# baoe/AlignGraph

Measured on AMD Instinct MI355X. Metric: aligned reads/sec through graph build+extend, higher is better.
Workload: dtype u32

## Files before the change

### aligngraph_amd/csrc/agx_core.h

```cpp
#pragma once
#include <stdint.h>
#include "../../include/agx.h"

#if defined(__HIPCC__)
#define AGX_HD __host__ __device__ __forceinline__
#else
#define AGX_HD inline
#endif

typedef uint32_t agx_u32;
typedef uint16_t agx_u16;
typedef uint8_t agx_u8;

#define AGX_NONE 0xFFFFFFFFu
#define AGX_TILE 64u
#ifndef AGX_REGION_TILES
#define AGX_REGION_TILES 32u
#endif
#define AGX_REGION_PAD 32u
#ifndef AGX_MAXV_LDS
#define AGX_MAXV_LDS 2u
#endif
#ifndef AGX_SWEEP_FIRST
#define AGX_SWEEP_FIRST 1
// ... 95 lines not shown
AGX_HD agx_u32 agx_cside_nruns(agx_u32 c) { return (c & 0xFFu) | (c >> 8) << 16; }
AGX_HD agx_u32 agx_cside_total(agx_u32 nruns) { return (nruns & 0xFFFFu) + (nruns >> 16); }
AGX_HD agx_wside agx_cside_rebuild(agx_u32 first, agx_u32 before, agx_u32 nruns) { const agx_u32 n1 = nruns & 0xFFFFu, r1 = first + before; return agx_wside{n1 ? r1 : 0u, (nruns >> 16) ? r1 + n1 : 0u, nruns}; }
AGX_HD bool agx_cside_in_order(const agx_wside &sd, unsigned long long &at) {
    const agx_u32 n1 = sd.nruns & 0xFFFFu, n2 = sd.nruns >> 16;
    const bool fine = sd.runs1 == (n1 ? at : 0ull) && sd.runs2 == (n2 ? at + n1 : 0ull);
    at += n1 + n2;
    return fine && at <= 0xFFFFFFFFull;
}
AGX_HD agx_u32 agx_cside_first(const agx_wside *sides, size_t n) { return !n ? 0u : (sides[0].nruns & 0xFFFFu) ? sides[0].runs1 : (sides[0].nruns >> 16) ? sides[0].runs2 : 0u; }
AGX_HD bool agx_sides_consecutive(const agx_wside *sides, size_t n, agx_u32 &first) {
    first = agx_cside_first(sides, n);
    unsigned long long at = first;
    for (size_t i = 0; i < n; i++) if (!agx_cside_in_order(sides[i], at)) return false;
    return true;
}
struct agx_refx { agx_u32 pos, len, byte; };
AGX_HD agx_u32 agx_ref_code(agx_u32 c) { return c == 'A' ? 0u : c == 'C' ? 1u : c == 'G' ? 2u : c == 'T' ? 3u : 4u; }
AGX_HD char agx_ref_base(agx_u32 code) { return (char)((0x54474341u >> (8u * (code & 3u))) & 0xFFu); }

struct agx_cmkey { agx_u32 cid, coff; };
struct agx_cmhead { agx_u32 cid, coff, n, start; };


enum { AGX_HF_AREV = 1, AGX_HF_SKIP = 2, AGX_HF_BNONE = 4 };

struct agx_dhit {
    agx_u32 a_t0, b_t0;
    agx_u32 a_runs, b_runs;
    agx_u32 a_slot;
// ... 1210 lines not shown
```

### aligngraph_amd/csrc/agx_engine.cpp

```cpp
#include "agx_unit.h"


struct HsaCopy {
    bool ok = false; hsa_agent_t cpu{}; std::vector<hsa_agent_t> gpu; std::vector<std::string> uuid;
    static hsa_status_t on_agent(hsa_agent_t a, void *p) {
        HsaCopy *H = (HsaCopy *)p; hsa_device_type_t t;
        if (hsa_agent_get_info(a, HSA_AGENT_INFO_DEVICE, &t) != HSA_STATUS_SUCCESS) return HSA_STATUS_SUCCESS;
        if (t == HSA_DEVICE_TYPE_CPU && !H->cpu.handle) H->cpu = a;
        if (t == HSA_DEVICE_TYPE_GPU) {
            char id[32] = {0};
            (void)hsa_agent_get_info(a, (hsa_agent_info_t)HSA_AMD_AGENT_INFO_UUID, id);
            H->gpu.push_back(a); H->uuid.push_back(std::string(id, strnlen(id, 21)));
        }
        return HSA_STATUS_SUCCESS;
    }
    HsaCopy() {
        if (getenv("AGX_NO_SDMA_DOWNLOAD")) return;
        if (hsa_init() != HSA_STATUS_SUCCESS) return;
        if (hsa_iterate_agents(on_agent, this) != HSA_STATUS_SUCCESS) return;
        ok = cpu.handle != 0 && !gpu.empty();
    }
    bool agent_of(int device, hsa_agent_t &out) const {
        static std::mutex m; static int known[64]; static hsa_agent_t agent[64];
        std::lock_guard<std::mutex> l(m);
// ... 265 lines not shown
        u->side_first = agx_cside_first(sd, n); unsigned long long at = u->side_first;
        for (size_t i = 0; i < n && fine; i++) { fine = agx_cside_in_order(sd[i], at); listed += agx_cside_pack(sd[i].nruns) == AGX_CS_ESC; }
        const size_t counts_bytes = (n * 2 + 7) & ~(size_t)7, bytes = n * 2 + listed * sizeof(agx_cside_esc);
        if (fine && bytes >= n * sizeof(agx_wside)) fine = false;
        if (fine) {
            u->s_csides.alloc(counts_bytes + (listed + 1) * sizeof(agx_cside_esc));
            agx_u16 *c = (agx_u16 *)u->s_csides.p; agx_cside_esc *l = (agx_cside_esc *)(u->s_csides.p + counts_bytes);
            u->wire_listed = l; u->n_csesc = listed;
            for (size_t i = 0; i < n; i++) { const agx_u32 v = agx_cside_pack(sd[i].nruns); c[i] = (agx_u16)v; if (v == AGX_CS_ESC) *l++ = agx_cside_esc{(agx_u32)i, sd[i].nruns}; }
        }
        if (getenv("AGX_LOAD_TIMING")) fprintf(stderr, "[agx load] compact side records: %.1f ms, 12 -> %.2f bytes per side, %.2f %% listed%s\n", now_ms() - t0, (double)bytes / n,
                                              100.0 * listed / n, fine ? "" : ": not used (the run pool is not in side order, or nothing gained)");
    }
    if (!fine) { u->s_csides.release(); return; }
    u->sides_compact = true;
}

void stage_tiled(agx_unit *u, unsigned threads) {
    u->tiled = false; u->n_other_t = 0; u->slot_row.clear(); u->n_win = 1;
    const size_t nh = u->nh, s4 = u->stride / 4;
    if (u->rows_diffed || getenv("AGX_NO_TILED_UPLOAD") || nh == 0 || u->n_rows == 0) { u->s_hits_t.release(); u->s_codes_t.release(); u->s_other_t.release(); return; }
    const double t0 = now_ms();
    const bool compact = want_compact();
    if (compact) u->s_hits_t.alloc_plain(nh + 1); else u->s_hits_t.alloc(nh + 1);
    u->s_codes_t.alloc(nh * s4 + 16); u->slot_row.resize(nh);
    const agx_whit *wh = u->s_hits.p; const agx_wside *sd = u->s_sides.p; const agx_wrun *wr = u->s_runs.p; const agx_u32 *perm = u->s_perm.p;
    const size_t n_rows = u->n_rows; std::vector<agx_u8> has_other((n_rows + 7) / 8, 0);
    for (size_t j = 0; j < u->n_other; j++) { const size_t r = (size_t)(u->s_other.p[j] / u->stride); if (r < n_rows) has_other[r >> 3] |= (agx_u8)(1u << (r & 7)); }
    auto idx0 = [&](const agx_whit &w) -> agx_u32 {
        if (!(w.flags & AGX_WF_RUNS1)) return w.a;
// ... 47 lines not shown
    const char *env = getenv("AGX_ROW_DIFF");
    const size_t n_pos = u->V.n_pos ? u->V.n_pos : u->T.ref.size();
    if (!env || atoi(env) == 0) return;
    const double t0 = now_ms();
    RowDiffs D;
    if (!build_row_diffs(u->s_hits_t.p, u->nh, u->s_sides.p, u->n_sides, u->s_runs.p, u->n_runs, u->s_codes_t.p, u->nh, u->stride, (const agx_u32 *)u->s_ref.p, n_pos, threads, D, true)) return;
    if (D.n_units * 2 + D.cnt.size() + (D.block_off.size() + D.block_first.size() + D.anchor_bits.size()) * 4 >= u->nh * (u->stride / 4)) return;
    adopt_row_diffs(u, D, threads);
    if (getenv("AGX_LOAD_TIMING")) fprintf(stderr, "[agx load] tile-ordered rows against the reference: %.1f ms, %zu rows (%zu as they are), %.1f -> %.1f bytes per row\n", now_ms() - t0, u->nh, u->n_rows_explicit,
                                          (double)(u->stride / 4), (double)(u->n_units * 2 + u->n_rowcnt + (u->n_blockoff + u->n_blockfirst + u->n_anchor) * 4) / u->nh);
}

void finish_staging(agx_unit *u, unsigned threads_rows, unsigned threads) {
    stage_rows(u, threads_rows);
    stage_order(u, threads);
    stage_tiled(u, threads);
    if (!u->tiled) stage_wire_hits(u, threads);
    stage_wire_sides(u);
    stage_rows_tiled(u, threads);
    u->V.slot_row = u->tiled ? u->slot_row.data() : nullptr;
    reserve_landing(u);
    u->staged = true; u->consumed = false; u->uploaded = false; u->built = false; u->downloaded = false;
}

void stage_inputs(agx_unit *u) {
    if (!u->have_ref || !u->have_threads) throw Error{E_ARG, "reference and contig threads must be set before upload"};
    if (u->consumed && u->pairs_staged) throw Error{E_ARG, "one-shot unit: its staged read alignments were overwritten by the download; load the unit again"};
    const double t0 = now_ms();
    HIP_OK(hipSetDevice(u->prm.device));
    u->cache_map.reset(); u->reads_map.reset();
    const size_t n_pos = u->T.ref.size();
    if (n_pos == 0 || n_pos >= 0xFFFFFF00ull) throw Error{E_ARG, "unit sequence is empty or too long"};
    if (u->T.cm_cnt.size() != n_pos) throw Error{E_ARG, "conti-mer chains were not built"};
    { size_t el = 0; for (const agx_cmseg &g : u->T.segs) el += g.len; if (el != u->T.n_cm) throw Error{E_ARG, "conti-mer runs were not built"}; }
// ... 260 lines not shown
    if (u->prm.flags & AGX_FLAG_KEEP_COUNTS) t(u->d_counts, (size_t)cap * 6);
    if (u->prm.flags & AGX_FLAG_EDGE_SUPPORT) t(u->d_e_cnt, (size_t)cap * AGX_MAXE);
    t(u->d_a_str, ids_cap + 1); t(u->d_a_meta, ids_cap + 16); t(u->d_a_mark, ids_cap + 2); t(u->d_side_xpos, (size_t)cap + 1);
    t(u->d_sp_bits, n_words + 1); t(u->d_sp_cnt, n_words + 1); t(u->d_sp_rank, n_words + 2);
    const size_t nb = (std::max<size_t>(n_pos, n_words) + 1 + 1023) / 1024;
    t(u->d_scan_tmp, 2 * (nb + 1) + 2 * ((nb + 1023) / 1024 + 1) + 16); t(u->d_scan_desc, 3 * scan_desc_of(u, cap));
}
template <class U> void fixed_bufs(U *u, Take &t) {
    const size_t n_pos = u->V.n_pos, nh = u->nh, n_tiles = tiles_of(u), n_regions = regions_of(u);
    t(u->d_cm_start, n_pos + 2); t(u->d_cm, u->n_cm + 1); t(u->d_ref, n_pos + 16); t(u->d_cm_head, n_pos + 1);
    t(u->d_segs, u->n_segs + 1); t(u->d_cntruns, u->n_cntruns + 1); t(u->d_cntchunks, u->n_cntchunks + 1); t(u->d_segchunks, u->n_segchunks + 1); t(u->d_segindex, u->n_segindex + 1);
    t(u->d_runs, u->n_runs + 1); t(u->d_vcodes, codes_bytes(u) * 4 + 16); t(u->d_other, others_up(u) + 1);
    if (u->rows_diffed) { t(u->d_units, u->n_units + 2); t(u->d_rowcnt, u->n_rowcnt); t(u->d_blockoff, u->n_blockoff); t(u->d_blockfirst, u->n_blockfirst); t(u->d_anchor, u->n_anchor); }
    else t(u->d_codes, codes_bytes(u) + 16);
    if (u->hits_compact) { t(u->d_chits, u->n_cblocks + 1); t(u->d_cesc, u->n_cesc + 1); t(u->d_cext, u->n_cext + 1); }
    if (u->sides_compact) { t(u->d_csides, u->n_sides + 1); t(u->d_csesc, u->n_csesc + 1); t(u->d_cside_scan, agx_side_scan_words(u->n_sides)); }
    t(u->d_whits, nh + 1); t(u->d_wsides, u->n_sides + 1); t(u->d_wruns, u->n_runs + 1); t(u->d_jump, u->n_jump + 1);
    if (u->ref_packed) { t(u->d_wref, (n_pos + 3) / 4 + 32); t(u->d_refx, u->n_refx + 1); }
    t(u->d_dhit, nh + 1);
    t(u->d_perm, nh + 1); t(u->d_tfirst, n_tiles + 2); t(u->d_ckey, nh + 1); t(u->d_long, AGX_LONG_MAX);
    t(u->d_tile_cnt, n_tiles + 1); t(u->d_tile_off, n_tiles + 2); t(u->d_cursor, n_tiles + 1);
    t(u->d_words, W_TOTAL);
    t(u->d_chain_end, (size_t)u->n_chain_end + 1);
    t(u->d_node_start, n_pos); t(u->d_node_cnt, n_pos); t(u->d_pos_succ, n_pos); t(u->d_slow_list, n_pos + 64);
    t(u->d_side_pk, n_pos + 2); t(u->d_tile_side, n_tiles + 2); t(u->d_tile_side_start, n_tiles + 2);
    t(u->d_big_list, n_tiles + 1); t(u->d_mid_list, n_tiles + 1);
    t(u->d_scratch, (size_t)AGX_BIG_WAVES * AGX_NF * AGX_MAXV_BIG * 64);
    t(u->d_region_off, n_regions + 1); t(u->d_pool_cnt, n_regions * AGX_REGION_PAD);
    if (u->prm.flags & AGX_FLAG_EDGE_SUPPORT) t(u->d_sup_tot, 2 * n_tiles + 2);
}
template <class U> void list_bufs(U *u, agx_u32 cap, Take &t) { t.note(u->list_cap, cap); t(u->d_unsorted, (size_t)cap + 1); t(u->d_tile_recs, ((size_t)cap + 4) * 8); }
template <class U> void ovf_bufs(U *u, agx_u32 cap, Take &t) { t.note(u->ovf_cap, cap); t(u->d_ovf, cap); t(u->d_a_ovf, (size_t)cap + 1); if (u->prm.flags & AGX_FLAG_EDGE_SUPPORT) t(u->d_ovf_cnt, cap); }
// ... 53 lines not shown
        std::lock_guard<std::mutex> up_turn(turn.up_m);
        u->up_timed = u->ev.all;
        if (u->up_timed) HIP_OK(hipEventRecord(u->ev_up0, st));
        static const size_t chunk = getenv("AGX_UP_CHUNK_MB") ? (size_t)atoi(getenv("AGX_UP_CHUNK_MB")) << 20 : 0;
        size_t sent = 0;
        auto up = [&](void *dst, const void *src, size_t bytes) {
            for (size_t at = 0; at < bytes;) { const size_t m = chunk ? std::min(chunk, bytes - at) : bytes; HIP_OK(hipMemcpyAsync((char *)dst + at, (const char *)src + at, m, hipMemcpyHostToDevice, st)); at += m; }
            sent += bytes;
        };
        up(u->d_segs.p, u->s_segs.p, u->n_segs * sizeof(agx_cmseg)); up(u->d_cntruns.p, u->s_cntruns.p, u->n_cntruns * sizeof(agx_cntrun));
        up(u->d_cntchunks.p, u->s_cntchunks.p, u->n_cntchunks * sizeof(agx_chunk)); up(u->d_segchunks.p, u->s_segchunks.p, u->n_segchunks * sizeof(agx_chunk)); up(u->d_segindex.p, u->s_segindex.p, u->n_segindex * 4);
        if (u->hits_compact) { up(u->d_chits.p, u->s_wire.p, u->n_cblocks * sizeof(agx_chit_block)); up(u->d_cesc.p, u->wire_esc, u->n_cesc * sizeof(agx_whit)); up(u->d_cext.p, u->wire_ext, u->n_cext * 4); }
        else up(u->d_whits.p, !u->tiled ? (const void *)u->s_hits.p : u->s_wire.p ? (const void *)u->s_wire.p : (const void *)u->s_hits_t.p, nh * sizeof(agx_whit));
        if (u->sides_compact) { up(u->d_csides.p, u->s_csides.p, u->n_sides * 2); up(u->d_csesc.p, u->wire_listed, u->n_csesc * sizeof(agx_cside_esc)); }
        else up(u->d_wsides.p, u->s_sides.p, u->n_sides * sizeof(agx_wside));
        up(u->d_wruns.p, u->s_runs.p, u->n_runs * sizeof(agx_wrun)); up(u->d_jump.p, u->s_jump_at.p, u->n_jump * 4);
        if (!u->tiled) up(u->d_perm.p, u->s_perm.p, nh * 4);
        up(u->d_tfirst.p, u->s_tfirst.p, ((size_t)u->n_tiles + 2) * 4);
        HIP_OK(hipEventRecord(u->ev_hits, st));
        auto small = [&] {
            up(u->d_other.p, u->tiled ? u->s_other_t.p : u->s_other.p, others_up(u) * 8);
            if (u->ref_packed) { up(u->d_wref.p, u->s_ref.p, (n_pos + 3) / 4); up(u->d_refx.p, u->s_refx.p, u->n_refx * sizeof(agx_refx)); } else up(u->d_ref.p, u->s_ref.p, n_pos);
            up(u->d_chain_end.p, u->s_chain_end.p, (size_t)u->n_chain_end * 4);
            layout_regions(u, nullptr, u->pool_cap - spill_min(u), true, st, &sent);
        };
        auto tables = [&] { up(u->d_blockoff.p, u->s_blockoff.p, u->n_blockoff * 4); up(u->d_blockfirst.p, u->s_blockfirst.p, u->n_blockfirst * 4); up(u->d_anchor.p, u->s_anchor.p, u->n_anchor * 4); };
        if (u->tiled) {
            small();
            if (u->rows_diffed) tables();
            const size_t s4 = u->stride / 4;
            for (agx_u32 w = 0; w < u->n_win; w++) {
// ... 97 lines not shown
        if (attempt > 8) throw Error{E_DEVICE, "build did not converge"};
        const size_t ids_cap = (size_t)n_pos + u->pool_cap;

        const double tb0 = now_ms();
        const bool early = !u->expanded && attempt == 0 && !u->ev.all;
        HIP_OK(wait_event(early ? u->ev_hits : u->ev_uploaded));
        trace(u, "build: wait for upload", tb0, n_pos);
        const double tb1 = now_ms();
        DeviceTurn &turn = turn_of(u->prm.device);
        std::unique_lock<std::mutex> my_turn(turn.m);
        st = turn.front;
        if (turn.n) HIP_OK(hipStreamWaitEvent(st, (u->ev.all || turn.prev_exclusive) ? turn.build_done[(turn.n - 1) & 1] : turn.sweep_done[(turn.n - 1) & 1], 0));
        if (u->ev.all) HIP_OK(hipEventRecord(u->ev.first, st));
        if (!u->expanded) {
            if (u->hits_compact) agx_launch_expand_hits(u->d_chits.p, u->d_cesc.p, u->d_cext.p, u->d_whits.p, nh, u->maxlen, st);
            if (u->sides_compact) agx_launch_expand_sides(u->d_csides.p, u->d_csesc.p, (agx_u32)u->n_csesc, u->d_wsides.p, (agx_u32)u->n_sides, u->side_first, u->d_cside_scan.p, st);
            agx_launch_expand_runs(u->d_wruns.p, u->d_runs.p, (agx_u32)u->n_runs, st);
            agx_launch_cm_tables(u->d_cntruns.p, u->d_cntchunks.p, (agx_u32)u->n_cntchunks, u->d_segs.p, u->d_segchunks.p, (agx_u32)u->n_segchunks, u->d_cm_start.p, u->d_cm.p, u->d_cm_head.p, n_pos, (agx_u32)u->n_cm, st);
        }
        {
            agx_zero_args Z; memset(&Z, 0, sizeof Z);
            auto seg = [&](int i, agx_u32 *ptr, size_t words) { Z.p[i] = ptr; Z.n[i] = (agx_u32)words; };
            seg(0, u->d_words.p, W_TOTAL); seg(1, u->d_tile_cnt.p, (size_t)u->n_tiles + 1); seg(2, u->d_cursor.p, (size_t)u->n_tiles + 1);
            seg(3, u->d_pool_cnt.p, (size_t)u->n_regions * AGX_REGION_PAD); seg(4, u->d_tile_side.p + u->n_tiles, 1); seg(5, u->d_sp_cnt.p, (size_t)u->n_words + 1);
            seg(6, reinterpret_cast<agx_u32 *>(u->d_scan_desc.p), 6 * u->scan_desc_n); seg(7, reinterpret_cast<agx_u32 *>(u->d_sp_bits.p), 2 * ((size_t)u->n_words + 1));
            agx_launch_zero(&Z, st);
            HIP_OK(hipMemsetAsync(u->d_a_mark.p, 0, ids_cap + 2, st));
        }
        u->ev.begin(); u->ev.mark(B_START, st);
        agx_prep_args PA{(const agx_whit *)u->d_whits.p, (const agx_wside *)u->d_wsides.p, u->d_runs.p, u->d_dhit.p, nh, u->prm.k, n_pos, u->d_tile_cnt.p, u->d_words.p + W_ERR,
                         u->d_perm.p, u->d_tfirst.p, u->d_ckey.p, u->lookback, u->d_long.p, u->d_words.p + W_LONGCOUNT, u->tiled ? 1u : 0u, u->d_perm.p};
        agx_launch_hit_prep(&PA, st);
// ... 929 lines not shown
```

### aligngraph_amd/csrc/agx_kargs.h

```cpp
#pragma once
#include <hip/hip_runtime_api.h>
#include "agx_core.h"

struct agx_prep_args {
    const agx_whit *whits; const agx_wside *sides;
    const agx_run *runs; agx_dhit *dhit; agx_u32 n_hits, k, n_pos;
    agx_u32 *tile_cnt;
    agx_u32 *err;
    const agx_u32 *perm, *tile_first; agx_u32 *ckey; agx_u32 lookback; agx_u32 *long_list, *long_count;
    agx_u32 tiled; agx_u32 *perm_out;
};

struct agx_bin_args { const agx_dhit *dhit; agx_u32 n_hits; const agx_u32 *tile_off; agx_u32 *cursor; agx_u32 *unsorted; agx_u32 cap;
                      const agx_u32 *long_count; };

struct agx_node_kargs {
    agx_sweep_args S;
    agx_u32 tile_lo, tile_hi;
    agx_u32 *pool_cnt;
    const agx_u32 *region_off;
    agx_u32 spill_lo; agx_u32 *spill_cnt;
    agx_u32 *mid_count; agx_u32 *mid_list;
    agx_u32 *big_count; agx_u32 *big_list;
    agx_u32 fallback_queued;
// ... 130 lines not shown
#define AGX_SLOW_WAVES 8192u

extern "C" {
struct agx_zero_args { agx_u32 *p[8]; agx_u32 n[8]; };
void agx_launch_zero(const agx_zero_args *, hipStream_t);
void agx_launch_cm_tables(const void *cnt_runs, const void *cnt_chunks, agx_u32 n_cnt_chunks, const agx_cmseg *segs, const void *seg_chunks, agx_u32 n_seg_chunks,
                           agx_u32 *cm_start, agx_cmkey *cm, agx_cmhead *head, agx_u32 n_pos, agx_u32 n_cm, hipStream_t);
void agx_launch_expand_codes(const void *packed, void *vcodes, size_t n_bases16, const unsigned long long *other, size_t n_other, hipStream_t);
void agx_launch_expand_rows(const void *whits, agx_u32 nh, const void *wsides, const void *wruns, const agx_u32 *anchor_bits, const agx_u32 *block_first, const agx_u8 *cnt, const agx_u32 *block_off,
                            const agx_u16 *units, const void *wref, void *vcodes, agx_u32 n_rows, agx_u32 stride, const unsigned long long *other, size_t n_other, hipStream_t);
void agx_launch_patch_codes(const unsigned long long *other, size_t n_other, void *vcodes, hipStream_t);
void agx_launch_expand_runs(const void *wruns, agx_run *runs, agx_u32 n_runs, hipStream_t);
void agx_launch_expand_hits(const agx_chit_block *blocks, const void *esc, const agx_u32 *ext, void *whits, agx_u32 nh, agx_u32 maxlen, hipStream_t);
inline size_t agx_side_scan_words(size_t n) { const size_t nb = (n + 1 + 4095) / 4096, nb2 = (nb + 4095) / 4096; return 2 * (n + 1) + 2 * (nb + 1) + 2 * (nb2 + 1); }
void agx_launch_expand_sides(const agx_u16 *counts, const agx_cside_esc *list, agx_u32 n_list, void *sides, agx_u32 n, agx_u32 first, agx_u32 *scan, hipStream_t);
void agx_launch_expand_ref(const void *packed, void *ref, size_t n_pos16, const void *refx, agx_u32 n_refx, hipStream_t);
void agx_launch_hit_prep(const agx_prep_args *, hipStream_t);
void agx_launch_exclusive_scan(const agx_u32 *in, agx_u32 *out, agx_u32 n, agx_u32 *tmp, hipStream_t);
void agx_launch_exclusive_scan1(const agx_u32 *in, agx_u32 *out, agx_u32 n, unsigned long long *desc, hipStream_t);
void agx_launch_exclusive_scan1_capped(const agx_u32 *in, agx_u32 *out, agx_u32 n, unsigned long long *desc, agx_u32 grid_cap, hipStream_t);
agx_u32 agx_scan_grid_limit(agx_u32 grid_cap);
void agx_launch_bin_fill(const agx_bin_args *, hipStream_t);
struct agx_fill_args { const agx_u32 *tile_off, *tile_first, *perm, *ckey; const agx_dhit *dhit; const agx_run *runs; void *recs; agx_u32 *scratch ;
                       agx_u32 n_tiles, cap, k, lookback; const agx_u32 *long_list, *long_count; agx_u32 *err;
                       agx_u32 *status; agx_u32 dense_queued; };
void agx_launch_tile_fill(const agx_fill_args *, hipStream_t);
void agx_launch_tile_sort(const agx_fill_args *, hipStream_t);
void agx_launch_node_sweep(const agx_node_kargs *, hipStream_t);
void agx_launch_node_sweep_big(const agx_node_kargs *, hipStream_t);
void agx_launch_edge_sweep(const agx_edge_kargs *, hipStream_t);
// ... 42 lines not shown
```

### aligngraph_amd/csrc/agx_kernels.hip

```cpp
#include <hip/hip_runtime.h>
#include "agx_kargs.h"

#define AGX_WAVES_PER_BLOCK 4
static_assert(AGX_MAXV_LDS <= AGX_EM_W && AGX_MAXV_MID <= AGX_EM_W, "the LDS sweep writes the x -> x+1 edges of every position it finishes: its buckets must fit the edge matrix");
#define AGX_XCDS 8u
#ifndef AGX_SWEEP_WAVES
#define AGX_SWEEP_WAVES 1
#endif

#define AGX_RETURN_IF_ABORTED(word) do { if (__builtin_amdgcn_readfirstlane((int)*(word)) != 0) return; } while (0)

__global__ void __launch_bounds__(256) agx_k_cm_layout(const agx_cntrun *runs, const agx_chunk *chunks, agx_u32 *cm_start, agx_cmhead *head, agx_u32 n_pos, agx_u32 n_cm) {
    const agx_chunk c = chunks[blockIdx.x];
    const agx_cntrun r = runs[c.run];
    const agx_u32 n = r.len - c.off < AGX_CM_CHUNK ? r.len - c.off : AGX_CM_CHUNK;
    for (agx_u32 j = threadIdx.x; j < n; j += 256u) agx_cm_layout_pos(r, c.off + j, cm_start, head);
    if (blockIdx.x == 0 && threadIdx.x == 0) { cm_start[n_pos] = n_cm; head[n_pos] = agx_cmhead{AGX_NONE, AGX_NONE, 0u, 0u}; }
}
__global__ void __launch_bounds__(256) agx_k_cm_fill(const agx_cmseg *segs, const agx_chunk *chunks, const agx_u32 *cm_start, agx_cmkey *cm, agx_cmhead *head) {
    const agx_chunk c = chunks[blockIdx.x];
    const agx_cmseg g = segs[c.run];
    const agx_u32 n = g.len - c.off < AGX_CM_CHUNK ? g.len - c.off : AGX_CM_CHUNK;
    for (agx_u32 j = threadIdx.x; j < n; j += 256u) agx_cm_fill_elem(g, c.off + j, cm_start, cm, head);
}
// ... 76 lines not shown
    if (escaped) { whits[i] = esc[B->esc + (agx_u32)__popcll(em & front)]; return; }
    const agx_whit w = agx_chit_decode(num, word, B->base, maxlen, side ? ext[B->ext + (agx_u32)__popcll(xm & front)] : 0u);
    whits[i] = make_uint4(w.a, w.b, w.row, (agx_u32)w.len | (agx_u32)w.flags << 16 | (agx_u32)w.back << 24);
}
__global__ void __launch_bounds__(256) agx_k_side_counts(const agx_u16 *counts, agx_wside *sides, agx_u32 *total, agx_u32 n) {
    const agx_u32 i = blockIdx.x * 256u + threadIdx.x;
    if (i < n) { const agx_u32 nr = agx_cside_nruns(counts[i]); sides[i].nruns = nr; total[i] = agx_cside_total(nr); }
}
__global__ void __launch_bounds__(256) agx_k_side_listed(const agx_cside_esc *list, agx_u32 n_list, agx_wside *sides, agx_u32 *total) {
    const agx_u32 j = blockIdx.x * 256u + threadIdx.x;
    if (j < n_list) { const agx_cside_esc e = list[j]; sides[e.side].nruns = e.nruns; total[e.side] = agx_cside_total(e.nruns); }
}
__global__ void __launch_bounds__(256) agx_k_side_firsts(const agx_u32 *before, agx_wside *sides, agx_u32 n, agx_u32 first) {
    const agx_u32 i = blockIdx.x * 256u + threadIdx.x;
    if (i < n) sides[i] = agx_cside_rebuild(first, before[i], sides[i].nruns);
}
__global__ void __launch_bounds__(256) agx_k_expand_ref(const agx_u32 *packed, uint4 *ref, size_t n16) {
    const size_t i = (size_t)blockIdx.x * 256u + threadIdx.x;
    if (i >= n16) return;
    const agx_u32 v = packed[i];
    agx_u32 w[4];
    for (int j = 0; j < 4; j++) { agx_u32 o = 0; for (int b = 0; b < 4; b++) o |= (agx_u32)(agx_u8)agx_ref_base((v >> (8 * j + 2 * b)) & 3u) << (8 * b); w[j] = o; }
    ref[i] = make_uint4(w[0], w[1], w[2], w[3]);
}
__global__ void __launch_bounds__(256) agx_k_patch_ref(const agx_refx *x, agx_u8 *ref) {
    const agx_refx r = x[blockIdx.x];
    for (agx_u32 j = threadIdx.x; j < r.len; j += 256u) ref[(size_t)r.pos + j] = (agx_u8)r.byte;
}

__global__ void __launch_bounds__(256) agx_k_hit_prep(agx_prep_args A) {
// ... 924 lines not shown
}
void agx_launch_expand_runs(const void *wruns, agx_run *runs, agx_u32 n_runs, hipStream_t st) {
    if (n_runs) hipLaunchKernelGGL(agx_k_expand_runs, dim3((n_runs + 255) / 256), dim3(256), 0, st, (const agx_wrun *)wruns, runs, n_runs);
}
void agx_launch_expand_hits(const agx_chit_block *blocks, const void *esc, const agx_u32 *ext, void *whits, agx_u32 nh, agx_u32 maxlen, hipStream_t st) {
    if (nh) hipLaunchKernelGGL(agx_k_expand_hits, dim3((nh + 255) / 256), dim3(256), 0, st, blocks, (const uint4 *)esc, ext, (uint4 *)whits, nh, maxlen);
}
void agx_launch_expand_sides(const agx_u16 *counts, const agx_cside_esc *list, agx_u32 n_list, void *sides, agx_u32 n, agx_u32 first, agx_u32 *scan, hipStream_t st) {
    if (!n) return;
    agx_u32 *total = scan, *before = scan + n + 1, *tmp = before + n + 1;
    hipLaunchKernelGGL(agx_k_side_counts, dim3((n + 255) / 256), dim3(256), 0, st, counts, (agx_wside *)sides, total, n);
    if (n_list) hipLaunchKernelGGL(agx_k_side_listed, dim3((n_list + 255) / 256), dim3(256), 0, st, list, n_list, (agx_wside *)sides, total);
    agx_launch_exclusive_scan(total, before, n, tmp, st);
    hipLaunchKernelGGL(agx_k_side_firsts, dim3((n + 255) / 256), dim3(256), 0, st, before, (agx_wside *)sides, n, first);
}
void agx_launch_expand_ref(const void *packed, void *ref, size_t n_pos16, const void *refx, agx_u32 n_refx, hipStream_t st) {
    const size_t n16 = n_pos16 / 16;
    if (n16) hipLaunchKernelGGL(agx_k_expand_ref, dim3((unsigned)((n16 + 255) / 256)), dim3(256), 0, st, (const agx_u32 *)packed, (uint4 *)ref, n16);
    if (n_refx) hipLaunchKernelGGL(agx_k_patch_ref, dim3(n_refx), dim3(256), 0, st, (const agx_refx *)refx, (agx_u8 *)ref);
}
void agx_launch_hit_prep(const agx_prep_args *A, hipStream_t st) {
    if (A->n_hits) hipLaunchKernelGGL(agx_k_hit_prep, dim3((A->n_hits + 255) / 256), dim3(256), 0, st, *A);
}

void agx_launch_exclusive_scan(const agx_u32 *in, agx_u32 *out, agx_u32 n, agx_u32 *tmp, hipStream_t st) {
    const agx_u32 m = n + 1;
    const agx_u32 nb = (m + AGX_SCAN_BLOCK - 1) / AGX_SCAN_BLOCK;
    if (nb == 1) { hipLaunchKernelGGL(agx_k_scan_blocks, dim3(1), dim3(256), 0, st, in, out, (agx_u32 *)nullptr, m); return; }
    agx_u32 *sums = tmp, *sums_scanned = tmp + nb + 1;
    hipLaunchKernelGGL(agx_k_scan_blocks, dim3(nb), dim3(256), 0, st, in, out, sums, m);
// ... 116 lines not shown
```

### aligngraph_amd/csrc/agx_unit.h

```cpp
#pragma once
#include <hip/hip_runtime_api.h>
#include <hsa/hsa.h>
#include <hsa/hsa_ext_amd.h>
#include <fcntl.h>
#include <sys/stat.h>
#include <unistd.h>

#include <algorithm>
#include <chrono>
#include <cstdio>
#include <cstdlib>
#include <cstring>
#include <memory>
#include <string>
#include <mutex>
#include <system_error>
#include <thread>
#include <type_traits>
#include <pthread.h>
#include <atomic>
#include <condition_variable>
#include <functional>
#include <vector>

// ... 89 lines not shown
    bool pending_walk = false;
    bool trimmed = false;
    bool expanded = false;
    hipEvent_t ev_built = nullptr;
    UnitOutput out; OutBuf out_initial; bool out_ready = false;
    UnitHelper helper;
    hsa_signal_t dl_signal{}; hsa_agent_t dl_agent{}; bool dl_sdma = false;
    enum { DL_SIGNALS = AGX_DL_PIECES + 2 };
    hsa_signal_t dl_piece[DL_SIGNALS] = {}; bool dl_piece_made = false, dl_streaming = false; agx_cut_args cuts{}; agx_u32 cut_main[AGX_DL_PIECES + 1] = {}, cut_side[AGX_DL_PIECES + 1] = {};
    double dl_t0 = 0, dl_est_ms = 0; size_t dl_stream_bytes = 0; std::atomic<bool> dl_timed{false};
    DevArena arena;
    PBuf<agx_whit> s_hits; PBuf<agx_wside> s_sides; PBuf<agx_wrun> s_runs; PBuf<agx_u8> s_codes; PBuf<unsigned long long> s_other; PBuf<agx_u32> s_jump; size_t n_other = 0, n_sides = 0, n_jump = 0;
    PBuf<agx_u8> s_ref; PBuf<agx_refx> s_refx; size_t n_refx = 0; bool ref_packed = false;
    PBuf<agx_u32> s_chain_end, s_region_off; PBuf<agx_cmseg> s_segs; size_t n_segs = 0;
    PBuf<agx_whit> s_hits_t; PBuf<agx_u8> s_codes_t; PBuf<unsigned long long> s_other_t; size_t n_other_t = 0; bool tiled = false; std::vector<agx_u32> slot_row;
    PBuf<char> s_wire, s_csides; const agx_whit *wire_esc = nullptr; const agx_u32 *wire_ext = nullptr; const agx_cside_esc *wire_listed = nullptr; size_t n_cblocks = 0, n_cesc = 0, n_cext = 0, n_csesc = 0; agx_u32 side_first = 0; bool hits_compact = false, sides_compact = false;
    agx_u32 front_windows = 1;
    agx_u32 n_win = 1, win_tile[9] = {};
    hipEvent_t ev_rows[8] = {}, ev_win[8] = {}, ev_sw0[8] = {}, ev_sw1[8] = {};
    PBuf<agx_u32> s_perm, s_tfirst, s_jump_at; agx_u32 lookback = 2;
    PBuf<char> s_landing;
    PBuf<agx_cntrun> s_cntruns; PBuf<agx_chunk> s_cntchunks, s_segchunks; PBuf<agx_u32> s_segindex; size_t n_cntruns = 0, n_cntchunks = 0, n_segchunks = 0, n_segindex = 0;
    PBuf<agx_u16> s_units; PBuf<agx_u8> s_rowcnt; PBuf<agx_u32> s_blockoff, s_blockfirst, s_anchor; size_t n_units = 0, n_rowcnt = 0, n_blockoff = 0, n_blockfirst = 0, n_anchor = 0, n_rows_explicit = 0; bool rows_diffed = false;
    size_t nh = 0, n_runs = 0, n_cm = 0, n_codes = 0; agx_u32 maxlen = 0;
    std::vector<agx_u32> row_slot;
    std::vector<uint64_t> row_off;
    std::shared_ptr<agx::ReadsIndex> reads_keep;
    std::unique_ptr<agx::FileView> reads_map;
    bool pairs_staged = false;
    agx::PairsFile pairs_file;
    DBuf<agx_u32> d_cm_start; DBuf<agx_cmkey> d_cm; DBuf<agx_cmhead> d_cm_head; DBuf<char> d_ref; DBuf<agx_cmseg> d_segs;
    DBuf<agx_run> d_runs; DBuf<agx_u8> d_codes, d_vcodes; DBuf<unsigned long long> d_other;
    DBuf<agx_u16> d_units; DBuf<agx_u8> d_rowcnt; DBuf<agx_u32> d_blockoff, d_blockfirst, d_anchor;
    DBuf<agx_cntrun> d_cntruns; DBuf<agx_chunk> d_cntchunks, d_segchunks; DBuf<agx_u32> d_jump, d_segindex;
    DBuf<agx_chit_block> d_chits; DBuf<agx_whit> d_cesc; DBuf<agx_u32> d_cext, d_cside_scan; DBuf<agx_u16> d_csides; DBuf<agx_cside_esc> d_csesc;
    DBuf<agx_whit> d_whits; DBuf<agx_wside> d_wsides; DBuf<agx_wrun> d_wruns; DBuf<agx_u8> d_wref; DBuf<agx_refx> d_refx;
    DBuf<agx_dhit> d_dhit; DBuf<agx_u32> d_tile_cnt, d_tile_off, d_cursor, d_unsorted, d_tile_recs, d_scan_tmp, d_words; DBuf<unsigned long long> d_scan_desc; size_t scan_desc_n = 0;
    agx_u32 pool_cap = 0, spill_lo = 0, ovf_cap = 0, list_cap = 0, sp_cap = 0;
    DBuf<agx_u32> d_pool_cnt, d_region_off; agx_u32 n_regions = 0;
    DBuf<agx_u32> d_node_start, d_slow_list, d_perm, d_tfirst, d_ckey, d_long; DBuf<agx_u16> d_node_cnt; DBuf<agx_u8> d_pos_succ;
    DBuf<agx_u32> d_cid, d_coff, d_cid0, d_coff0, d_off0, d_next; DBuf<agx_u8> d_base, d_flags; DBuf<agx_sref> d_sref; DBuf<int> d_counts;
    DBuf<agx_u32> d_e_cnt, d_ovf_cnt, d_sup_tot, d_lsup;
    bool support_valid = false; uint64_t sup_events = 0, sup_adds = 0;
    DBuf<char> d_ut;
    DBuf<agx_edge_ovf> d_ovf; DBuf<agx_u32> d_mid_list, d_big_list, d_scratch, d_huge_list, d_scratch_huge; bool huge = false, dense = false;
    agx_u32 n_ids = 0;
    DBuf<agx_u32> d_side_pk, d_tile_side, d_tile_side_start, d_aid_of; DBuf<char> d_a_str;
    DBuf<agx_u8> d_a_meta, d_a_mark; DBuf<agx_walknode> d_fetch, d_sp_node; DBuf<agx_u32> d_a_nid; DBuf<agx_edge_ovf> d_a_ovf; agx_compact_args walk_args{};
    DBuf<agx_u32> d_chain_end, d_side_xpos, d_sp_cnt, d_sp_rank; DBuf<unsigned long long> d_sp_bits;
    agx_u32 n_chain_end = 0, n_special = 0, n_words = 0;
// ... 55 lines not shown
```

Baseline: 1.482 billion.

## Delta-encode run records for upload and expand sides and runs in one kernel

```diff
diff --git a/aligngraph_amd/csrc/agx_core.h b/aligngraph_amd/csrc/agx_core.h
--- a/aligngraph_amd/csrc/agx_core.h
+++ b/aligngraph_amd/csrc/agx_core.h
@@ -133,6 +133,55 @@
     unsigned long long at = first;
     for (size_t i = 0; i < n; i++) if (!agx_cside_in_order(sides[i], at)) return false;
     return true;
+}
+#define AGX_CR_BLOCK 64u
+struct agx_crun_block { agx_u32 runs, units, esc, listed; };
+AGX_HD agx_u32 agx_crun_units(agx_u32 k) { return k ? k + 2u : 0u; }
+AGX_HD agx_u32 agx_crun_side_units(agx_u32 nruns, bool listed) { return listed ? 0u : agx_crun_units(nruns & 0xFFFFu) + agx_crun_units(nruns >> 16); }
+AGX_HD bool agx_crun_escaped(agx_u32 head) { return (head & 0xFFu) == 0; }
+AGX_HD bool agx_crun_encode(const agx_wrun *r, agx_u32 k, agx_u16 *out) {
+    bool fits = r[0].q < 256u && r[0].n >= 1u && r[0].n < 256u;
+    for (agx_u32 j = 1; j < k && fits; j++) {
+        const agx_u32 dq = (agx_u32)r[j].q - ((agx_u32)r[j - 1].q + r[j - 1].n), dt = r[j].t - (r[j - 1].t + r[j - 1].n);
+        fits = dq < 16u && dt < 16u && r[j].n >= 1u && r[j].n < 256u;
+        if (fits) out[2 + j] = (agx_u16)(dq << 12 | dt << 8 | r[j].n);
+    }
+    if (!fits) { for (agx_u32 j = 0; j < k + 2u; j++) out[j] = 0; return false; }
+    out[0] = (agx_u16)(r[0].t & 0xFFFFu); out[1] = (agx_u16)(r[0].t >> 16); out[2] = (agx_u16)((agx_u32)r[0].q << 8 | r[0].n);
+    return true;
+}
+AGX_HD agx_u32 agx_crun_decode(const agx_u16 *in, const agx_wrun *esc, agx_u32 k, agx_run *out) {
+    const agx_u32 head = in[2];
+    if (agx_crun_escaped(head)) { for (agx_u32 j = 0; j < k; j++) { const agx_wrun r = esc[j]; out[j] = agx_run{r.q, r.t, r.n}; } return k; }
+    agx_u32 q = head >> 8, t = (agx_u32)in[0] | (agx_u32)in[1] << 16, n = head & 0xFFu;
+    out[0] = agx_run{q, t, n};
+    for (agx_u32 j = 1; j < k; j++) {
+        const agx_u32 w = in[2 + j];
+        q += n + (w >> 12); t += n + ((w >> 8) & 15u); n = w & 0xFFu;
+        out[j] = agx_run{q, t, n};
+    }
+    return 0;
+}
+AGX_HD void agx_crun_pack_side(const agx_wrun *r, agx_u32 nruns, bool listed, agx_u16 *units, agx_u32 &nu, agx_wrun *esc, agx_u32 &ne) {
+    const agx_u32 k[2] = {nruns & 0xFFFFu, nruns >> 16};
+    nu = ne = 0;
+    for (int m = 0; m < 2; m++) {
+        if (!k[m]) continue;
+        if (listed || !agx_crun_encode(r, k[m], units + nu)) { for (agx_u32 j = 0; j < k[m]; j++) esc[ne++] = r[j]; }
+        if (!listed) nu += agx_crun_units(k[m]);
+        r += k[m];
+    }
+}
+AGX_HD agx_u32 agx_crun_side_escaped(const agx_u16 *units, agx_u32 nruns, bool listed) {
+    const agx_u32 k1 = nruns & 0xFFFFu, k2 = nruns >> 16;
+    if (listed) return k1 + k2;
+    return (k1 && agx_crun_escaped(units[2]) ? k1 : 0u) + (k2 && agx_crun_escaped(units[agx_crun_units(k1) + 2u]) ? k2 : 0u);
+}
+AGX_HD void agx_crun_unpack_side(const agx_u16 *units, const agx_wrun *esc, agx_u32 nruns, bool listed, agx_run *out) {
+    const agx_u32 k1 = nruns & 0xFFFFu, k2 = nruns >> 16;
+    if (listed) { for (agx_u32 j = 0; j < k1 + k2; j++) { const agx_wrun r = esc[j]; out[j] = agx_run{r.q, r.t, r.n}; } return; }
+    if (k1) esc += agx_crun_decode(units, esc, k1, out);
+    if (k2) agx_crun_decode(units + agx_crun_units(k1), esc, k2, out + k1);
 }
 struct agx_refx { agx_u32 pos, len, byte; };
 AGX_HD agx_u32 agx_ref_code(agx_u32 c) { return c == 'A' ? 0u : c == 'C' ? 1u : c == 'G' ? 2u : c == 'T' ? 3u : 4u; }
diff --git a/aligngraph_amd/csrc/agx_engine.cpp b/aligngraph_amd/csrc/agx_engine.cpp
--- a/aligngraph_amd/csrc/agx_engine.cpp
+++ b/aligngraph_amd/csrc/agx_engine.cpp
@@ -303,6 +303,63 @@
     }
     if (!fine) { u->s_csides.release(); return; }
     u->sides_compact = true;
+}
+void release_wire_runs(agx_unit *u) { u->runs_compact = false; u->n_crblocks = u->n_cresc = u->n_crunits = 0; u->wire_resc = nullptr; u->wire_runits = nullptr; u->s_cruns.release(); }
+inline bool want_row_diffs() { const char *e = getenv("AGX_ROW_DIFF"); return e && atoi(e) != 0; }
+inline bool want_compact_runs() { const char *e = getenv("AGX_WIRE_RUNS_PLAIN"); return !(e && atoi(e) != 0); }
+void stage_wire_runs(agx_unit *u, unsigned threads) {
+    release_wire_runs(u);
+    const size_t n = u->n_sides, n_runs = u->n_runs;
+    if (!u->sides_compact || !want_compact_runs() || u->rows_diffed || want_row_diffs() || n == 0 || n_runs == 0 || u->side_first != 0) return;
+    const double t0 = now_ms();
+    const size_t n_blocks = (n + AGX_CR_BLOCK - 1) / AGX_CR_BLOCK;
+    const unsigned T = (unsigned)std::max<size_t>(1, std::min<size_t>(std::min(threads, 16u), n_blocks));
+    const agx_wside *sd = u->s_sides.p; const agx_wrun *wr = u->s_runs.p;
+    std::vector<agx_crun_block> blocks(n_blocks); std::vector<std::vector<agx_u16>> units(T); std::vector<std::vector<agx_wrun>> esc(T);
+    std::vector<size_t> runs_of(T, 0), listed_of(T, 0);
+    auto first = [&](unsigned t) { return n_blocks * t / T; };
+    on_threads(T, [&](unsigned t) {
+        std::vector<agx_u16> &U = units[t]; std::vector<agx_wrun> &E = esc[t];
+        const size_t lo = first(t) * AGX_CR_BLOCK, hi = std::min<size_t>(n, first(t + 1) * AGX_CR_BLOCK);
+        if (lo >= hi) return;
+        size_t r0 = 0;
+        for (size_t i = lo; i < n; i++) if (sd[i].nruns) { r0 = agx_cside_first(sd + i, 1); break; }
+        size_t all_units = 0;
+        for (size_t i = lo; i < hi; i++) all_units += agx_crun_side_units(sd[i].nruns, agx_cside_pack(sd[i].nruns) == AGX_CS_ESC);
+        U.resize(all_units);
+        agx_u16 *u_at = U.data(); agx_wrun few[512];
+        size_t runs = 0, listed = 0;
+        for (size_t i = lo; i < hi; i++) {
+            if ((i & (AGX_CR_BLOCK - 1)) == 0) blocks[i / AGX_CR_BLOCK] = agx_crun_block{(agx_u32)runs, (agx_u32)(u_at - U.data()), (agx_u32)E.size(), (agx_u32)listed};
+            const agx_u32 nr = sd[i].nruns, tot = agx_cside_total(nr); const bool is_listed = agx_cside_pack(nr) == AGX_CS_ESC;
+            agx_u32 nu = 0, ne = 0;
+            if (is_listed) { const size_t e_at = E.size(); E.resize(e_at + tot); agx_crun_pack_side(wr + r0 + runs, nr, true, u_at, nu, E.data() + e_at, ne); }
+            else { agx_crun_pack_side(wr + r0 + runs, nr, false, u_at, nu, few, ne); if (ne) E.insert(E.end(), few, few + ne); }
+            u_at += nu; runs += tot; listed += is_listed;
+        }
+        runs_of[t] = runs; listed_of[t] = listed;
+    });
+    size_t nr = 0, nu = 0, ne = 0, nl = 0;
+    for (unsigned t = 0; t < T; t++) {
+        for (size_t b = first(t); b < first(t + 1); b++) { blocks[b].runs += (agx_u32)nr; blocks[b].units += (agx_u32)nu; blocks[b].esc += (agx_u32)ne; blocks[b].listed += (agx_u32)nl; }
+        nr += runs_of[t]; nu += units[t].size(); ne += esc[t].size(); nl += listed_of[t];
+    }
+    const size_t head = n_blocks * sizeof(agx_crun_block), bytes = head + ne * sizeof(agx_wrun) + nu * 2;
+    const bool fine = nr == n_runs && nu <= 0xFFFFFFFFull && bytes < n_runs * sizeof(agx_wrun);
+    if (fine) {
+        u->s_cruns.alloc(bytes + 16);
+        memcpy(u->s_cruns.p, blocks.data(), head);
+        agx_wrun *e_at = (agx_wrun *)(u->s_cruns.p + head); agx_u16 *u_at = (agx_u16 *)(e_at + ne);
+        u->wire_resc = e_at; u->wire_runits = u_at;
+        for (unsigned t = 0; t < T; t++) {
+            if (!esc[t].empty()) memcpy(e_at, esc[t].data(), esc[t].size() * sizeof(agx_wrun));
+            if (!units[t].empty()) memcpy(u_at, units[t].data(), units[t].size() * 2);
+            e_at += esc[t].size(); u_at += units[t].size();
+        }
+        u->n_crblocks = n_blocks; u->n_cresc = ne; u->n_crunits = nu; u->runs_compact = true;
+    }
+    if (getenv("AGX_LOAD_TIMING")) fprintf(stderr, "[agx load] compact run records: %.1f ms, 8 -> %.2f bytes per run, %.2f %% escaped%s\n", now_ms() - t0, (double)bytes / n_runs, 100.0 * ne / n_runs,
+                                          fine ? "" : ": not used (nothing gained, or runs of the pool that no side names)");
 }
 
 void stage_tiled(agx_unit *u, unsigned threads) {
@@ -380,10 +437,13 @@
 void finish_staging(agx_unit *u, unsigned threads_rows, unsigned threads) {
     stage_rows(u, threads_rows);
     stage_order(u, threads);
-    stage_tiled(u, threads);
-    if (!u->tiled) stage_wire_hits(u, threads);
-    stage_wire_sides(u);
+    const int device = u->prm.device;
+    on_threads(2, [&](unsigned t) {
+        if (t == 0) { stage_tiled(u, threads); if (!u->tiled) stage_wire_hits(u, threads); }
+        else { (void)hipSetDevice(device); stage_wire_sides(u); stage_wire_runs(u, 1); }
+    });
     stage_rows_tiled(u, threads);
+    if (u->rows_diffed) release_wire_runs(u);
     u->V.slot_row = u->tiled ? u->slot_row.data() : nullptr;
     reserve_landing(u);
     u->staged = true; u->consumed = false; u->uploaded = false; u->built = false; u->downloaded = false;
@@ -674,8 +734,10 @@
     if (u->rows_diffed) { t(u->d_units, u->n_units + 2); t(u->d_rowcnt, u->n_rowcnt); t(u->d_blockoff, u->n_blockoff); t(u->d_blockfirst, u->n_blockfirst); t(u->d_anchor, u->n_anchor); }
     else t(u->d_codes, codes_bytes(u) + 16);
     if (u->hits_compact) { t(u->d_chits, u->n_cblocks + 1); t(u->d_cesc, u->n_cesc + 1); t(u->d_cext, u->n_cext + 1); }
-    if (u->sides_compact) { t(u->d_csides, u->n_sides + 1); t(u->d_csesc, u->n_csesc + 1); t(u->d_cside_scan, agx_side_scan_words(u->n_sides)); }
-    t(u->d_whits, nh + 1); t(u->d_wsides, u->n_sides + 1); t(u->d_wruns, u->n_runs + 1); t(u->d_jump, u->n_jump + 1);
+    if (u->sides_compact) { t(u->d_csides, u->n_sides + 1); t(u->d_csesc, u->n_csesc + 1); if (!u->runs_compact) t(u->d_cside_scan, agx_side_scan_words(u->n_sides)); }
+    if (u->runs_compact) { t(u->d_crblocks, u->n_crblocks + 1); t(u->d_cresc, u->n_cresc + 1); t(u->d_crunits, u->n_crunits + 1); }
+    t(u->d_whits, nh + 1); t(u->d_wsides, u->n_sides + 1); if (!u->runs_compact) t(u->d_wruns, u->n_runs + 1);
+    t(u->d_jump, u->n_jump + 1);
     if (u->ref_packed) { t(u->d_wref, (n_pos + 3) / 4 + 32); t(u->d_refx, u->n_refx + 1); }
     t(u->d_dhit, nh + 1);
     t(u->d_perm, nh + 1); t(u->d_tfirst, n_tiles + 2); t(u->d_ckey, nh + 1); t(u->d_long, AGX_LONG_MAX);
@@ -759,7 +821,9 @@
         else up(u->d_whits.p, !u->tiled ? (const void *)u->s_hits.p : u->s_wire.p ? (const void *)u->s_wire.p : (const void *)u->s_hits_t.p, nh * sizeof(agx_whit));
         if (u->sides_compact) { up(u->d_csides.p, u->s_csides.p, u->n_sides * 2); up(u->d_csesc.p, u->wire_listed, u->n_csesc * sizeof(agx_cside_esc)); }
         else up(u->d_wsides.p, u->s_sides.p, u->n_sides * sizeof(agx_wside));
-        up(u->d_wruns.p, u->s_runs.p, u->n_runs * sizeof(agx_wrun)); up(u->d_jump.p, u->s_jump_at.p, u->n_jump * 4);
+        if (u->runs_compact) { up(u->d_crblocks.p, u->s_cruns.p, u->n_crblocks * sizeof(agx_crun_block)); up(u->d_cresc.p, u->wire_resc, u->n_cresc * sizeof(agx_wrun)); up(u->d_crunits.p, u->wire_runits, u->n_crunits * 2); }
+        else up(u->d_wruns.p, u->s_runs.p, u->n_runs * sizeof(agx_wrun));
+        up(u->d_jump.p, u->s_jump_at.p, u->n_jump * 4);
         if (!u->tiled) up(u->d_perm.p, u->s_perm.p, nh * 4);
         up(u->d_tfirst.p, u->s_tfirst.p, ((size_t)u->n_tiles + 2) * 4);
         HIP_OK(hipEventRecord(u->ev_hits, st));
@@ -887,8 +951,11 @@
         if (u->ev.all) HIP_OK(hipEventRecord(u->ev.first, st));
         if (!u->expanded) {
             if (u->hits_compact) agx_launch_expand_hits(u->d_chits.p, u->d_cesc.p, u->d_cext.p, u->d_whits.p, nh, u->maxlen, st);
-            if (u->sides_compact) agx_launch_expand_sides(u->d_csides.p, u->d_csesc.p, (agx_u32)u->n_csesc, u->d_wsides.p, (agx_u32)u->n_sides, u->side_first, u->d_cside_scan.p, st);
-            agx_launch_expand_runs(u->d_wruns.p, u->d_runs.p, (agx_u32)u->n_runs, st);
+            if (u->runs_compact) agx_launch_expand_sides_runs(u->d_csides.p, u->d_csesc.p, u->d_crblocks.p, u->d_crunits.p, u->d_cresc.p, u->d_wsides.p, u->d_runs.p, (agx_u32)u->n_sides, u->side_first, st);
+            else {
+                if (u->sides_compact) agx_launch_expand_sides(u->d_csides.p, u->d_csesc.p, (agx_u32)u->n_csesc, u->d_wsides.p, (agx_u32)u->n_sides, u->side_first, u->d_cside_scan.p, st);
+                agx_launch_expand_runs(u->d_wruns.p, u->d_runs.p, (agx_u32)u->n_runs, st);
+            }
             agx_launch_cm_tables(u->d_cntruns.p, u->d_cntchunks.p, (agx_u32)u->n_cntchunks, u->d_segs.p, u->d_segchunks.p, (agx_u32)u->n_segchunks, u->d_cm_start.p, u->d_cm.p, u->d_cm_head.p, n_pos, (agx_u32)u->n_cm, st);
         }
         {
diff --git a/aligngraph_amd/csrc/agx_kargs.h b/aligngraph_amd/csrc/agx_kargs.h
--- a/aligngraph_amd/csrc/agx_kargs.h
+++ b/aligngraph_amd/csrc/agx_kargs.h
@@ -168,6 +168,7 @@
 void agx_launch_expand_hits(const agx_chit_block *blocks, const void *esc, const agx_u32 *ext, void *whits, agx_u32 nh, agx_u32 maxlen, hipStream_t);
 inline size_t agx_side_scan_words(size_t n) { const size_t nb = (n + 1 + 4095) / 4096, nb2 = (nb + 4095) / 4096; return 2 * (n + 1) + 2 * (nb + 1) + 2 * (nb2 + 1); }
 void agx_launch_expand_sides(const agx_u16 *counts, const agx_cside_esc *list, agx_u32 n_list, void *sides, agx_u32 n, agx_u32 first, agx_u32 *scan, hipStream_t);
+void agx_launch_expand_sides_runs(const agx_u16 *counts, const agx_cside_esc *list, const agx_crun_block *blocks, const agx_u16 *units, const void *esc, void *sides, agx_run *runs, agx_u32 n, agx_u32 first, hipStream_t);
 void agx_launch_expand_ref(const void *packed, void *ref, size_t n_pos16, const void *refx, agx_u32 n_refx, hipStream_t);
 void agx_launch_hit_prep(const agx_prep_args *, hipStream_t);
 void agx_launch_exclusive_scan(const agx_u32 *in, agx_u32 *out, agx_u32 n, agx_u32 *tmp, hipStream_t);
diff --git a/aligngraph_amd/csrc/agx_kernels.hip b/aligngraph_amd/csrc/agx_kernels.hip
--- a/aligngraph_amd/csrc/agx_kernels.hip
+++ b/aligngraph_amd/csrc/agx_kernels.hip
@@ -114,6 +114,26 @@
 __global__ void __launch_bounds__(256) agx_k_side_firsts(const agx_u32 *before, agx_wside *sides, agx_u32 n, agx_u32 first) {
     const agx_u32 i = blockIdx.x * 256u + threadIdx.x;
     if (i < n) sides[i] = agx_cside_rebuild(first, before[i], sides[i].nruns);
+}
+__device__ __forceinline__ agx_u32 agx_wave_incl_scan(agx_u32 v, agx_u32 lane);
+__global__ void __launch_bounds__(256) agx_k_expand_sides_runs(const agx_u16 *counts, const agx_cside_esc *list, const agx_crun_block *blocks, const agx_u16 *units, const agx_wrun *esc,
+                                                               agx_wside *sides, agx_run *runs, agx_u32 n, agx_u32 first) {
+    const agx_u32 i = blockIdx.x * 256u + threadIdx.x, lane = threadIdx.x & 63u;
+    if (i - lane >= n) return;
+    const bool valid = i < n;
+    const agx_crun_block B = blocks[i >> 6];
+    const agx_u32 c = valid ? counts[i] : 0u;
+    const bool listed = c == AGX_CS_ESC;
+    const unsigned long long lm = __ballot(listed);
+    const agx_u32 nr = listed ? list[B.listed + (agx_u32)__popcll(lm & ((1ull << lane) - 1ull))].nruns : agx_cside_nruns(c);
+    const agx_u32 tot = agx_cside_total(nr), nu = agx_crun_side_units(nr, listed);
+    const agx_u32 r_at = B.runs + agx_wave_incl_scan(tot, lane) - tot;
+    const agx_u16 *mine = units + ((size_t)B.units + agx_wave_incl_scan(nu, lane) - nu);
+    const agx_u32 ne = agx_crun_side_escaped(mine, nr, listed);
+    const agx_u32 e_at = B.esc + agx_wave_incl_scan(ne, lane) - ne;
+    if (!valid) return;
+    sides[i] = agx_cside_rebuild(first, r_at, nr);
+    agx_crun_unpack_side(mine, esc + e_at, nr, listed, runs + (size_t)first + r_at);
 }
 __global__ void __launch_bounds__(256) agx_k_expand_ref(const agx_u32 *packed, uint4 *ref, size_t n16) {
     const size_t i = (size_t)blockIdx.x * 256u + threadIdx.x;
@@ -1068,6 +1088,9 @@
     agx_launch_exclusive_scan(total, before, n, tmp, st);
     hipLaunchKernelGGL(agx_k_side_firsts, dim3((n + 255) / 256), dim3(256), 0, st, before, (agx_wside *)sides, n, first);
 }
+void agx_launch_expand_sides_runs(const agx_u16 *counts, const agx_cside_esc *list, const agx_crun_block *blocks, const agx_u16 *units, const void *esc, void *sides, agx_run *runs, agx_u32 n, agx_u32 first, hipStream_t st) {
+    if (n) hipLaunchKernelGGL(agx_k_expand_sides_runs, dim3((n + 255) / 256), dim3(256), 0, st, counts, list, blocks, units, (const agx_wrun *)esc, (agx_wside *)sides, runs, n, first);
+}
 void agx_launch_expand_ref(const void *packed, void *ref, size_t n_pos16, const void *refx, agx_u32 n_refx, hipStream_t st) {
     const size_t n16 = n_pos16 / 16;
     if (n16) hipLaunchKernelGGL(agx_k_expand_ref, dim3((unsigned)((n16 + 255) / 256)), dim3(256), 0, st, (const agx_u32 *)packed, (uint4 *)ref, n16);
diff --git a/aligngraph_amd/csrc/agx_unit.h b/aligngraph_amd/csrc/agx_unit.h
--- a/aligngraph_amd/csrc/agx_unit.h
+++ b/aligngraph_amd/csrc/agx_unit.h
@@ -127,6 +127,7 @@
     PBuf<agx_u8> s_ref; PBuf<agx_refx> s_refx; size_t n_refx = 0; bool ref_packed = false;
     PBuf<agx_u32> s_chain_end, s_region_off; PBuf<agx_cmseg> s_segs; size_t n_segs = 0;
     PBuf<agx_whit> s_hits_t; PBuf<agx_u8> s_codes_t; PBuf<unsigned long long> s_other_t; size_t n_other_t = 0; bool tiled = false; std::vector<agx_u32> slot_row;
+    PBuf<char> s_cruns; const agx_wrun *wire_resc = nullptr; const agx_u16 *wire_runits = nullptr; size_t n_crblocks = 0, n_cresc = 0, n_crunits = 0; bool runs_compact = false;
     PBuf<char> s_wire, s_csides; const agx_whit *wire_esc = nullptr; const agx_u32 *wire_ext = nullptr; const agx_cside_esc *wire_listed = nullptr; size_t n_cblocks = 0, n_cesc = 0, n_cext = 0, n_csesc = 0; agx_u32 side_first = 0; bool hits_compact = false, sides_compact = false;
     agx_u32 front_windows = 1;
     agx_u32 n_win = 1, win_tile[9] = {};
@@ -147,6 +148,7 @@
     DBuf<agx_u16> d_units; DBuf<agx_u8> d_rowcnt; DBuf<agx_u32> d_blockoff, d_blockfirst, d_anchor;
     DBuf<agx_cntrun> d_cntruns; DBuf<agx_chunk> d_cntchunks, d_segchunks; DBuf<agx_u32> d_jump, d_segindex;
     DBuf<agx_chit_block> d_chits; DBuf<agx_whit> d_cesc; DBuf<agx_u32> d_cext, d_cside_scan; DBuf<agx_u16> d_csides; DBuf<agx_cside_esc> d_csesc;
+    DBuf<agx_crun_block> d_crblocks; DBuf<agx_wrun> d_cresc; DBuf<agx_u16> d_crunits;
     DBuf<agx_whit> d_whits; DBuf<agx_wside> d_wsides; DBuf<agx_wrun> d_wruns; DBuf<agx_u8> d_wref; DBuf<agx_refx> d_refx;
     DBuf<agx_dhit> d_dhit; DBuf<agx_u32> d_tile_cnt, d_tile_off, d_cursor, d_unsorted, d_tile_recs, d_scan_tmp, d_words; DBuf<unsigned long long> d_scan_desc; size_t scan_desc_n = 0;
     agx_u32 pool_cap = 0, spill_lo = 0, ovf_cap = 0, list_cap = 0, sp_cap = 0;
```

After: 1.412 billion. -4.8%, worse.
